# Arktis2022/Spiking-Diffusion

Measured on AMD Instinct MI355X. Metric: images/sec + LIF-kernel HBM GB/s, MNIST 100-step sample T=16, 1->8 GPU, higher is better.
Workload: dtype fp32-exact (4 fp6 digits x fp4 spikes on the block-scaled MFMA + certified decisions + exact 6-digit recomputation of flagged neurons)

## Files before the change

### spiking-diffusion_amd/csrc/den_mfma_fp6v2.hip

```cpp
#include "den_common.h"
#include "../../include/spkdiff.h"
#include <math.h>
#include <stdlib.h>
#include <type_traits>
#include <utility>

namespace {

typedef int v6i __attribute__((ext_vector_type(6)));
typedef int v8i __attribute__((ext_vector_type(8)));
typedef float v16f __attribute__((ext_vector_type(16)));

constexpr int T16 = 16;
constexpr int CK = 32;
constexpr int POSB = T16 * CK / 2;
constexpr int WT = 64 * 24;
constexpr int N_PAIR = 18;
constexpr int N_D4 = 5;
constexpr int N_MAIN = N_PAIR + N_D4;
constexpr int N_L5 = 2;
constexpr int NACC = 2;
constexpr int W_PIECES = (N_PAIR * WT + 1023) / 1024;
constexpr int W_LDS = W_PIECES * 1024;
constexpr int W_SLAB = ((N_MAIN + N_L5) * WT + 1023) / 1024 * 1024;

constexpr unsigned FLAG_CAP = 1u << 20;

struct V2Args {
  const uint8_t* in0; int nch;
  const uint8_t* wq; const double* scale; const double* bias; const float* wl1;
  const float* bn_a; const float* bn_b;
  uint8_t* out; uint8_t* out_cnt;
  unsigned* flags;
  unsigned flag_cap;
  long long ticket_idx;
  int handover;
  const int* qtab;
  const int* n_dyn;
  const uint8_t* need; const int* cls_cnt; const int* cls_list;
  int B, Cout, Cin;
  int gx, nsets;
};

#define SPK_FP6_PRE "s_nop 1\n\t"
#define SPK_MFMA2(CLS, acc, av, bv, sa, sb)                                                                          \
  asm volatile(SPK_FP6_PRE "v_mfma_scale_f32_32x32x64_f8f6f4 %0, %1, %2, %0, %3, %4 op_sel_hi:[0,0,0] cbsz:4 blgp:2"  \
               : "+" CLS(acc) : "v"(av), "v"(bv), "v"(sa), "v"(sb))
#define SPK_MFMA2_Z(CLS, acc, av, bv, sa, sb)                                                                        \
  asm volatile(SPK_FP6_PRE "v_mfma_scale_f32_32x32x64_f8f6f4 %0, %1, %2, 0, %3, %4 op_sel_hi:[0,0,0] cbsz:4 blgp:2"   \
               : "=&" CLS(acc) : "v"(av), "v"(bv), "v"(sa), "v"(sb))

constexpr int SPK_V2_KMIN = 2;
constexpr float SPK_V2_SPARE = 1.0f;
constexpr int SPK_V2_REC_STEP = 13;
constexpr int SPK_V2_LP_PAIRS = 1;
constexpr int SPK_V2_GX_KB = 2560;
constexpr int SPK_V2_HALF_FILL = 2;
constexpr int SPK_V2_LPS_MIN_B = 64;
constexpr int SPK_V2_LP_SPLIT_MAX = 512;
constexpr int SPK_V2_PF = 6;

constexpr float CERT_4EPS = 4.0f * 2.38418579e-07f;

__device__ __forceinline__ void store_tile_spikes(uint8_t* out, uint8_t* out_cnt, unsigned mybits, int lane, long long rec_base,
                                                  long long cnt_base, bool ok) {
  const unsigned bitsv = spk_transpose16_rows(mybits, lane);
  if (out_cnt && ok) out_cnt[cnt_base + (lane & 31)] = (uint8_t)__popc(mybits);
  if (ok) *reinterpret_cast<uint2*>(out + rec_base + (lane & 15) * 16 + 8 * ((lane >> 4) & 1)) = spk_e2m1_record(bitsv);
}

__device__ const uint8_t V2_HALF_REC[2][64] = {
    {0, 1, 2, 3, 4, 5, 6, 7, 8, 9, 10, 11, 12, 13, 14, 15, 16, 17, 18, 19, 20, 21, 22, 23,
     23, 23, 23, 23, 23, 23, 23, 23, 23, 23, 23, 23, 23, 23, 23, 23, 23, 23, 23, 23, 23, 23, 23, 23, 24},
    {24, 25, 26, 27, 28, 29, 30, 31, 32, 33, 34, 35, 36, 37, 38, 39, 40, 41, 42, 43, 44, 45, 46, 47,
     47, 47, 47, 47, 47, 47, 47, 47, 47, 47, 47, 47, 47, 47, 47, 47, 47, 47, 47, 47, 47, 47, 47, 47, 24}};

enum : int { V2_INT = 0, V2_TOP, V2_RIGHT, V2_LEFT, V2_BOTTOM, V2_NCLS };
struct V2Plan { int nblk; int tap[9]; int nt[9]; };
constexpr int V2_FT = 3;
constexpr V2Plan V2_PLAN[V2_NCLS] = {
    {9, {0, 1, 2, 3, 4, 5, 6, 7, 8}, {3, 3, 3, 3, 3, 3, 3, 3, 3}},
    {6, {3, 4, 5, 6, 7, 8}, {3, 3, 3, 3, 3, 3}},
    {6, {0, 1, 3, 4, 6, 7}, {3, 3, 3, 3, 3, 3}},
    {6, {1, 2, 4, 5, 7, 8}, {3, 3, 3, 3, 3, 3}},
    {9, {0, 6, 7, 8, 1, 2, 3, 4, 5}, {3, 1, 1, 1, 3, 3, 3, 3, 3}}};
constexpr V2Plan v2_uniform_plan(int nt) {
  V2Plan p = {9, {0, 1, 2, 3, 4, 5, 6, 7, 8}, {}};
  for (int b = 0; b < 9; ++b) p.nt[b] = nt;
  return p;
}
constexpr int v2_plan_start(const V2Plan& p, int blk) {
  int n = 0;
  for (int b = 0; b < blk; ++b) n += p.nt[b];
  return n;
}
constexpr int v2_plan_blk(const V2Plan& p, int s) {
  int b = 0;
  while (s >= p.nt[b]) s -= p.nt[b++];
  return b;
}
__device__ constexpr uint8_t V2_FULL_POS[8][V2_FT][2] = {
    {{0, 1}, {2, 3}, {4, 5}},       {{6, 13}, {20, 27}, {34, 41}},  {{7, 14}, {21, 28}, {35, 42}},  {{43, 44}, {45, 46}, {47, 40}},
    {{8, 9}, {10, 11}, {12, 15}},   {{16, 17}, {18, 19}, {22, 23}}, {{24, 25}, {26, 29}, {30, 31}}, {{32, 33}, {36, 37}, {38, 39}}};
__device__ constexpr uint8_t V2_WAVE_CLS[8] = {V2_TOP, V2_RIGHT, V2_LEFT, V2_BOTTOM, V2_INT, V2_INT, V2_INT, V2_INT};
constexpr bool v2_full_map_ok() {
  bool seen[48] = {};
  for (int w = 0; w < 8; ++w)
    for (int i = 0; i < V2_FT; ++i)
      for (int h = 0; h < 2; ++h) {
        const int p = V2_FULL_POS[w][i][h];
        if (p >= 48 || seen[p]) return false;
        seen[p] = true;
      }
  for (int w = 0; w < 8; ++w) {
    const V2Plan& pl = V2_PLAN[V2_WAVE_CLS[w]];
    for (int i = 0; i < V2_FT; ++i)
      for (int tap = 0; tap < 9; ++tap) {
        int n = 0;
        for (int b = 0; b < pl.nblk; ++b) n += pl.tap[b] == tap && i >= V2_FT - pl.nt[b];
        if (n > 1) return false;
        for (int h = 0; h < 2 && n == 0; ++h) {
          const int y = V2_FULL_POS[w][i][h] / 7 + tap / 3 - 1, x = V2_FULL_POS[w][i][h] % 7 + tap % 3 - 1;
          if (y >= 0 && y < 7 && x >= 0 && x < 7) return false;
        }
      }
  }
  return true;
}
static_assert(v2_full_map_ok(), "full 7x7 items: position table and block lists");

template <int H, int W, int NWV, bool SPLIT, int NTP, bool HALF = false, int CLS = V2_INT>
__device__ __forceinline__ void fp6v2_body(const V2Args& a, const int g, const int il, const int lanes, const int n_images,
                                           const int* __restrict__ slots) {
  constexpr bool PRUNE = NTP > 0;
  static_assert(!HALF || (PRUNE && !SPLIT && H == 7 && W == 7 && NWV == 4 && NTP == 3), "half-image items: 7x7, four waves x three tiles");
  constexpr bool REC = !PRUNE;
  constexpr int HW = H * W, PW = W + 1;
  constexpr int Hb = SPLIT ? H / 2 : H;
  constexpr int Hin = SPLIT ? Hb + 1 : H;
  constexpr int HWb = Hb * W;
  static_assert(SPLIT ? ((H % 2) == 0 && (HWb % (2 * NWV)) == 0)
                      : ((HW & 1) == 1 && ((HW / 2) % NWV) == 0), "whole 32-row tiles on every wave (+ one odd position)");
  static_assert(!PRUNE || (!SPLIT && (NWV == 4 || NWV == 8) && NTP <= (HWb / 2) / NWV), "position lists: 7x7 items");
  constexpr int NT = PRUNE ? NTP : (HWb / 2) / NWV;
  constexpr int N_AGPR = NWV == 4 ? (NACC * NT < 16 ? NACC * NT : 16) : 0;
  constexpr int NPP = (Hin + 2) * PW + 1;
  constexpr int A_BYTES = NPP * POSB;
  constexpr int PPR = (W + 3) / 4;
  constexpr int NA = Hin * PPR;
  constexpr int NPA = (NA + NWV - 1) / NWV;
  constexpr int NPW = (W_PIECES + NWV - 1) / NWV;
  constexpr bool BSKIP = NWV == 8 && !PRUNE && !SPLIT;
  static_assert(!BSKIP || (H == 7 && W == 7 && NT == V2_FT), "border skip: the position table is for 7x7 items of three tiles per wave");
  static_assert(BSKIP || CLS == V2_INT, "wave classes: full 7x7 items only");
  static_assert(NWV >= 8 || NACC * NT <= 16 || (NT - 1) * NACC <= N_AGPR + 2, "only the last tile may straddle the register files");
  constexpr bool AH = NWV == 8 && !PRUNE;
  constexpr int NBUF = 2;
  extern __shared__ __attribute__((aligned(16))) uint8_t lds[];
  uint8_t* const sA = lds;
  uint8_t* const sW = lds + NBUF * A_BYTES;
  int* const s_cin = reinterpret_cast<int*>(lds + NBUF * A_BYTES + NBUF * W_LDS);
  int* const s_row = s_cin + NPP * 16;
  int* const s_nmax = s_row + (HWb + 1) * 16;
  const unsigned sA_addr = spk_lds_addr(sA), sW_addr = sA_addr + NBUF * A_BYTES;
  const int tid = threadIdx.x, lane = tid & 63, wave = tid >> 6;
  const int nch = a.nch;
  const int G = a.Cout >> 5;
  for (int i = tid; i < NBUF * A_BYTES / 16; i += NWV * 64) reinterpret_cast<uint4*>(sA)[i] = make_uint4(0, 0, 0, 0);
  if (REC)
    for (int i = tid; i < NPP * 16; i += NWV * 64) s_cin[i] = 0;
  __syncthreads();

  const int row = lane & 31, half = lane >> 5;
  const int hsel = (row >> 2) & 1, tt = (row & 3) + 4 * (row >> 3);
  int a_off[NT];
  int p_out[NT];
#pragma unroll
  for (int i = 0; i < NT; ++i) {
    const int p = BSKIP ? (int)V2_FULL_POS[wave & 7][i % V2_FT][hsel] : 2 * (wave + NWV * i) + hsel;
    a_off[i] = ((p / W) * PW + (p % W)) * POSB + tt * 16;
    p_out[i] = BSKIP ? (int)V2_FULL_POS[wave & 7][i % V2_FT][half] : 2 * (wave + NWV * i) + half;
  }

  const int wave_s = __builtin_amdgcn_readfirstlane(wave);
  unsigned pa_pk[NPA];
#pragma unroll
  for (int j = 0; j < NPA; ++j) {
    int id = wave_s * NPA + j;
    id = id < NA ? id : NA - 1;
    const int y = id / PPR, px = id - y * PPR;
    const int np = (W - 4 * px) < 4 ? (W - 4 * px) : 4;
    const unsigned src = (unsigned)((y * W + 4 * px) * POSB), dst = (unsigned)(((y + 1) * PW + 1 + 4 * px) * POSB);
    pa_pk[j] = src | (dst << 14) | ((unsigned)(np - 1) << 29);
  }
  const unsigned lane16 = (unsigned)lane * 16u;
  const unsigned wave_k = (unsigned)wave_s * 1024u;
  auto issue_piece = [&](int q, const uint8_t* aslab, const uint8_t* wslab, unsigned dA, unsigned dW) {
    if (q < NPA) {
      const unsigned pk = pa_pk[q];
      const unsigned np = ((pk >> 29) & 3u) + 1u;
      const unsigned long long mask = np == 4 ? ~0ull : ((1ull << (16 * np)) - 1ull);
      spk_dma16s_masked(aslab + (pk & 0x3fffu), lane16, dA + ((pk >> 14) & 0x7fffu), mask);
    } else {
      unsigned ko = wave_k + 1024u * NWV * (unsigned)(q - NPA);
      if (NWV * (q - NPA) + NWV - 1 >= W_PIECES) ko = ko < (unsigned)W_PIECES * 1024u ? ko : ko - 1024u * NWV;
      spk_dma16s(wslab + ko, lane16, dW + ko);
    }
  };
  const uint8_t* const wbase = a.wq + (long long)g * nch * W_SLAB;
  auto aslab_of = [&](int itm, int c) -> const uint8_t* {
    const int b = HALF ? itm >> 1 : (PRUNE ? slots[itm] : (SPLIT ? itm >> 1 : itm)), band = SPLIT ? itm & 1 : 0;
    return a.in0 + ((long long)b * nch + c) * HW * POSB + band * (Hb - 1) * W * POSB;
  };
  const int nitems = (SPLIT || HALF) ? 2 * n_images : n_images;

  const int co = g * 32 + (lane & 31);
  const float scale_f = (float)a.scale[co], bias_f = (float)a.bias[co];
  const float bna = a.bn_a[co], bnb = a.bn_b[co];
  const float Bc = fmaf(bias_f, bna, bnb);
  const float cE = 2.0f * 2.38418579e-07f * (fabsf(bnb) + fabsf(Bc)) + 1e-30f;
  const float cT = 528.0f * scale_f * fabsf(bna) * 1.000001f;
  const float Ac4 = 1024.0f * scale_f * bna;

  const int sc_a = 0x7f7f7f7f;
  const int sc_p = half ? (int)0x82828282u : (int)0x87878787u;

  int it = 0;
  if (il < nitems) {
    const uint8_t* as0 = aslab_of(il, 0);
#pragma unroll
    for (int q = 0; q < NPA + NPW; ++q) issue_piece(q, as0, wbase, sA_addr, sW_addr);
    if constexpr (AH) {
      spk_dma_wait_all();
      __syncthreads();
    }
  }
  for (int itm = il; itm < nitems; itm += lanes) {
    const int b = HALF ? itm >> 1 : (PRUNE ? slots[itm] : (SPLIT ? itm >> 1 : itm)), band = SPLIT ? itm & 1 : 0;
    const int band_off = band * PW * POSB;
    int n_list = 2 * NT * NWV;
    if constexpr (PRUNE) {
      const uint8_t* rec = HALF ? &V2_HALF_REC[itm & 1][0] : a.need + (long long)b * 64;
      n_list = __builtin_amdgcn_readfirstlane((int)rec[48]);
#pragma unroll
      for (int i = 0; i < NT; ++i) {
        const int k2 = 2 * (wave + NWV * i);
        const int p = rec[k2 + hsel];
        a_off[i] = ((p / W) * PW + (p % W)) * POSB + tt * 16;
        p_out[i] = rec[k2 + half];
      }
    }
    v16f acc[NT][NACC];
    int cnt[NT];
#pragma unroll
    for (int i = 0; i < NT; ++i) cnt[i] = 0;
    constexpr int NREC = Hin * W * 16, NR = (NREC + NWV * 64 - 1) / (NWV * 64);
    int creg[NR];
    int rec_off[NR];
    bool rec_ok[NR];
#pragma unroll
    for (int k = 0; k < NR; ++k) {
      creg[k] = 0;
      const int r = tid + k * NWV * 64;
      const int cl = r >> 4, t = r & 15;
      rec_ok[k] = r < NREC;
      rec_off[k] = rec_ok[k] ? (((cl / W) + 1) * PW + 1 + (cl % W)) * POSB + t * 16 : 0;
    }
    constexpr int PFX = NWV == 4 ? SPK_V2_PF : 4;
    v6i bp[2][2];
    v4i af[PFX];
    for (int c = 0; c < nch; ++c, ++it) {
      const int buf = it & 1, buf1 = buf ^ 1;
      if constexpr (!AH) {
        spk_dma_wait_all();
        __syncthreads();
      }
      int nb = itm, nc = c + 1;
      if (nc == nch) { nc = 0; nb = itm + lanes; }
      const bool have_next = nb < nitems;
      const uint8_t* n_aslab = aslab_of(have_next ? nb : itm, have_next ? nc : c);
      const uint8_t* n_wslab = wbase + (long long)(have_next ? nc : c) * W_SLAB;
      const unsigned n_dA = sA_addr + buf1 * A_BYTES;
      const unsigned n_dW = sW_addr + buf1 * W_LDS;

      v4i rvq[NR];
      auto compute = [&](auto first_tag) {
        constexpr bool FIRST = decltype(first_tag)::value;
        const uint8_t* A = sA + buf * A_BYTES + band_off;
        const uint8_t* Wb = sW + buf * W_LDS;
        auto toff = [](int tap) constexpr -> int { return ((tap / 3) * PW + (tap % 3)) * POSB; };
        constexpr V2Plan P = BSKIP ? V2_PLAN[CLS] : v2_uniform_plan(NT);
        constexpr int NBLK = P.nblk, NSTEP = v2_plan_start(P, NBLK);
        constexpr int PF = PFX;
        constexpr int NPIECES = NPA + NPW;
        static_assert(P.nt[0] == NT, "the first block writes (not accumulates) every accumulator");
        static_assert(2 * NBLK >= NPIECES, "two copy slots per block: every DMA piece of the wave gets one");
        static_assert((!AH || NSTEP >= 2 * PF) && (!REC || NSTEP > SPK_V2_REC_STEP), "look-ahead slots; the record-count steps exist");
        static_assert(!AH || (v2_plan_start(P, (NPIECES + 1) / 2) <= NSTEP - PF && v2_plan_start(P, NBLK - 2) <= NSTEP - PF),
                      "chunk barrier behind the copies and the last weight-tile read");
        auto lda_at = [&](const uint8_t* base, auto s_tag) -> v4i {
          constexpr int s = decltype(s_tag)::value;
          constexpr int blk = v2_plan_blk(P, s), i = NT - P.nt[blk] + (s - v2_plan_start(P, blk));
          return *reinterpret_cast<const v4i*>(base + a_off[i] + toff(P.tap[blk]));
        };
        auto lda = [&](auto s_tag) -> v4i { return lda_at(A, s_tag); };
        auto ldb = [&](int tile) -> v6i {
          const uint8_t* p = Wb + tile * WT;
          const v4i x = *reinterpret_cast<const v4i*>(p + lane * 16);
          typedef const volatile __attribute__((address_space(3))) v2i* lds_v2i_ptr;
          const v2i y = *(lds_v2i_ptr)SPK_LDS(p + 1024 + lane * 8);
          const v6i r = {x[0], x[1], x[2], x[3], y[0], y[1]};
          return r;
        };
        if constexpr (!AH || FIRST) {
          bp[0][0] = ldb(2 * P.tap[0]); bp[0][1] = ldb(2 * P.tap[0] + 1);
          static_for<PF>([&](auto s_tag) { af[decltype(s_tag)::value] = lda(s_tag); });
        }
        const uint8_t* An = sA + buf1 * A_BYTES + band_off;
        const uint8_t* Wn = sW + buf1 * W_LDS;
        const bool ahead = AH && c + 1 < nch;
        static_for<NSTEP>([&](auto s_tag) {
          constexpr int s = decltype(s_tag)::value;
          constexpr int blk = v2_plan_blk(P, s), nt = P.nt[blk], j = s - v2_plan_start(P, blk);
          constexpr int i = NT - nt + j;
          if constexpr (AH && s == NSTEP - PF) {
            asm volatile("s_waitcnt vmcnt(0)\n\ts_barrier" ::: "memory");
          }
          const v4i av = af[s % PF];
          if constexpr (s + PF < NSTEP) af[s % PF] = lda(std::integral_constant<int, s + PF>{});
          else if constexpr (AH) {
            constexpr int k = s % PF;
            if (ahead) af[k] = lda_at(An, std::integral_constant<int, k>{});
          }
#define V2_DMA_SLOT()                                                                              \
  do {                                                                                             \
    if constexpr (j == 0 && 2 * blk < NPIECES) issue_piece(2 * blk, n_aslab, n_wslab, n_dA, n_dW);     \
    if constexpr (j == (nt > 1 ? nt / 2 : 0) && 2 * blk + 1 < NPIECES)                             \
      issue_piece(2 * blk + 1, n_aslab, n_wslab, n_dA, n_dW);                                      \
  } while (0)
#define V2_NEXT_TILES()                                                                            \
  do {                                                                                             \
    if constexpr (j == 0 && blk + 1 < NBLK) {                                                      \
      bp[(blk + 1) & 1][0] = ldb(2 * P.tap[(blk + 1) % 9]);                                        \
      bp[(blk + 1) & 1][1] = ldb(2 * P.tap[(blk + 1) % 9] + 1);                                    \
    }                                                                                              \
  } while (0)
          if constexpr (!REC) {
            asm volatile("v_bcnt_u32_b32 %0, %1, %0\n\tv_bcnt_u32_b32 %0, %2, %0\n\tv_bcnt_u32_b32 %0, %3, %0\n\t"
                         "v_bcnt_u32_b32 %0, %4, %0" : "+v"(cnt[i]) : "v"(av[0]), "v"(av[1]), "v"(av[2]), "v"(av[3]));
          }
#define V2_PAIR_MFMA(J)                                                                                      \
do {                                                                                                        \
  if constexpr (FIRST && blk == 0) {                                                                        \
    if constexpr (NACC * i + (J) < N_AGPR) SPK_MFMA2_Z("a", acc[i][J], av, bp[0][J], sc_a, sc_p);              \
    else SPK_MFMA2_Z("v", acc[i][J], av, bp[0][J], sc_a, sc_p);                                             \
  } else {                                                                                                  \
    if constexpr (NACC * i + (J) < N_AGPR) SPK_MFMA2("a", acc[i][J], av, bp[blk & 1][J], sc_a, sc_p);          \
    else SPK_MFMA2("v", acc[i][J], av, bp[blk & 1][J], sc_a, sc_p);                                         \
  }                                                                                                         \
} while (0)
          V2_PAIR_MFMA(0);
          __builtin_amdgcn_sched_barrier(0);
          V2_DMA_SLOT();
          V2_NEXT_TILES();
          if constexpr (REC) {
            if constexpr (s == 1) {
#pragma unroll
              for (int k = 0; k < NR; ++k) rvq[k] = *reinterpret_cast<const v4i*>(sA + buf * A_BYTES + rec_off[k]);
            }
            if constexpr (s == SPK_V2_REC_STEP) {
#pragma unroll
              for (int k = 0; k < NR; ++k)
                creg[k] += __builtin_popcount((unsigned)rvq[k][0]) + __builtin_popcount((unsigned)rvq[k][1]) +
                           __builtin_popcount((unsigned)rvq[k][2]) + __builtin_popcount((unsigned)rvq[k][3]);
            }
          }
          V2_PAIR_MFMA(1);
          __builtin_amdgcn_sched_barrier(0);
          if constexpr (AH && s == NSTEP - 1) {
            if (ahead) {
              auto ldb_n = [&](int tile) -> v6i {
                const uint8_t* p = Wn + tile * WT;
                const v4i x = *reinterpret_cast<const v4i*>(p + lane * 16);
                typedef const volatile __attribute__((address_space(3))) v2i* lds_v2i_ptr;
                const v2i y = *(lds_v2i_ptr)SPK_LDS(p + 1024 + lane * 8);
                const v6i r = {x[0], x[1], x[2], x[3], y[0], y[1]};
                return r;
              };
              bp[0][0] = ldb_n(2 * P.tap[0]); bp[0][1] = ldb_n(2 * P.tap[0] + 1);
            }
          }
        });
      };
      if (c == 0) compute(std::true_type{}); else compute(std::false_type{});
    }

    if constexpr (REC) {
#pragma unroll
      for (int k = 0; k < NR; ++k)
        if (rec_ok[k]) s_cin[(rec_off[k] / POSB) * 16 + ((rec_off[k] % POSB) >> 4)] = creg[k];
      if (tid <= HWb) s_nmax[tid] = 0;
      __syncthreads();
      for (int e = tid; e < HWb * 16; e += NWV * 64) {
        const int pp = e >> 4, t = e & 15;
        const int* c0 = s_cin + (((pp / W) + band) * PW + (pp % W)) * 16 + t;
        int sum = 0;
#pragma unroll
        for (int dy = 0; dy < 3; ++dy)
#pragma unroll
          for (int dx = 0; dx < 3; ++dx) sum += c0[(dy * PW + dx) * 16];
        s_row[e] = sum;
        atomicMax(&s_nmax[pp], sum);
      }
      __syncthreads();
    }
    asm volatile("s_nop 15\n\ts_nop 15" ::: "memory");

#pragma unroll
    for (int k = 0; k < NT; ++k) {
      const int i = k == 0 ? NT - 1 : k - 1;
#pragma unroll
      for (int j = 0; j < NACC; ++j)
        if (NACC * i + j < N_AGPR) asm volatile("" : "+a"(acc[i][j]));
      float v = 0.f;
      unsigned mybits = 0;
      bool flg = false;
      int cntv[16];
      if constexpr (!REC) {
#pragma unroll
        for (int r = 0; r < 16; ++r) {
          const int rowA = (r & 3) + 8 * (r >> 2);
          const int c0 = __builtin_amdgcn_readlane(cnt[i], rowA), c1 = __builtin_amdgcn_readlane(cnt[i], rowA + 4);
          cntv[r] = half ? c1 : c0;
        }
      }
      int nmax_rec = 0;
      if constexpr (REC) nmax_rec = s_nmax[BSKIP ? p_out[i] : 2 * (wave + NWV * i) + half];
      typedef float v2f __attribute__((ext_vector_type(2)));
      float zmax = 0.f, dmin = 3.0e38f;
      int nmax = nmax_rec;
#pragma unroll
      for (int r2 = 0; r2 < 16; r2 += 2) {
        const v2f p0 = {acc[i][0][r2], acc[i][0][r2 + 1]}, p1 = {acc[i][1][r2], acc[i][1][r2 + 1]};
        const v2f q4 = __builtin_elementwise_fma(p0, (v2f){1024.0f, 1024.0f}, p1);
        const v2f z2 = __builtin_elementwise_fma(q4, (v2f){Ac4, Ac4}, (v2f){Bc, Bc});
        if constexpr (!REC) nmax = max(nmax, max(cntv[r2], cntv[r2 + 1]));
#pragma unroll
        for (int e = 0; e < 2; ++e) {
          const float z = z2[e];
          zmax = fmaxf(zmax, fabsf(z));
          const float h = fmaf(z - v, 0.5f, v);
          const float hm = h - 1.0f;
          dmin = fminf(dmin, fabsf(hm));
          const bool s = h >= 1.0f;
          v = s ? 0.0f : h;
          mybits = __builtin_amdgcn_alignbit(mybits, __float_as_uint(hm), 31);
        }
      }
      mybits = ~(__builtin_bitreverse32(mybits) >> 16) & 0xffffu;
      flg = dmin <= SPK_V2_SPARE * fmaf(zmax, 2.5f * CERT_4EPS, fmaf((float)nmax, cT, cE));
      if (__builtin_amdgcn_ballot_w64(flg) != 0ull) {
        float v2 = 0.f, dh = 0.f;
        bool f2 = false;
        if constexpr (REC) {
          const v4i* rp = reinterpret_cast<const v4i*>(s_row + (BSKIP ? p_out[i] : 2 * (wave + NWV * i) + half) * 16);
#pragma unroll
          for (int q = 0; q < 4; ++q) {
            const v4i c4 = rp[q];
            cntv[4 * q] = c4[0]; cntv[4 * q + 1] = c4[1]; cntv[4 * q + 2] = c4[2]; cntv[4 * q + 3] = c4[3];
          }
        }
#pragma unroll
        for (int r2 = 0; r2 < 16; r2 += 2) {
          const v2f p0 = {acc[i][0][r2], acc[i][0][r2 + 1]}, p1 = {acc[i][1][r2], acc[i][1][r2 + 1]};
          const v2f q4 = __builtin_elementwise_fma(p0, (v2f){1024.0f, 1024.0f}, p1);
          const v2f z2 = __builtin_elementwise_fma(q4, (v2f){Ac4, Ac4}, (v2f){Bc, Bc});
#pragma unroll
          for (int e = 0; e < 2; ++e) {
            const float z = z2[e];
            const float ct = fmaf((float)cntv[r2 + e], cT, cE);
            dh = fmaf(fabsf(z) + fabsf(v2), 0.625f * CERT_4EPS, fmaf(dh, 0.5f, 0.5f * ct));
            const float h = fmaf(z - v2, 0.5f, v2);
            f2 = f2 || (fabsf(h - 1.0f) <= SPK_V2_SPARE * dh);
            v2 = h >= 1.0f ? 0.0f : h;
          }
        }
        flg = flg && f2;
      }
      const int ti = wave + NWV * i;
      const int p = (PRUNE || BSKIP) ? p_out[i] : 2 * ti + half + band * HWb;
      const bool listed = !PRUNE || 2 * ti + half < n_list;
      if (flg && listed) {
        const long long n = ((long long)b * a.Cout + co) * HW + p;
        const unsigned idx = atomicAdd(a.flags, 1u);
        if (idx < a.flag_cap) a.flags[2 + idx] = (unsigned)n;
        else atomicOr(a.flags + 2 + FLAG_CAP + (n >> 5), 1u << (n & 31));
      }
      const long long rec = (((long long)b * G + g) * HW + p) * POSB;
      store_tile_spikes(a.out, a.out_cnt, mybits, lane, rec, (((long long)b * G + g) * HW + p) * 32, listed);
      __builtin_amdgcn_sched_barrier(0);
    }
  }
  spk_dma_wait_all();
}

__device__ __forceinline__ void fp6v2_wg_map(const V2Args& a, int& g, int& il, int& lanes) {
  const int k = blockIdx.x, G = a.Cout >> 5;
  if (a.gx > 0) {
    const int S = gridDim.x >> 3, x = k & 7, slot = k >> 3;
    const int npart = 8 / a.nsets, set = x % a.nsets, xi = x / a.nsets, lanes_x = S / a.gx;
    g = set * a.gx + slot % a.gx;
    il = xi * lanes_x + slot / a.gx;
    lanes = npart * lanes_x;
  } else {
    g = k % G;
    il = k / G;
    lanes = gridDim.x / G;
  }
}

__device__ __forceinline__ void fp6v2_handover(const V2Args& a) {
  if (!a.handover) return;
  __syncthreads();
  if (threadIdx.x == 0) {
    if (atomicAdd(a.flags + a.ticket_idx, 1u) == gridDim.x - 1) {
      a.flags[1] = atomicAdd(a.flags, 0u);
      a.flags[0] = 0u;
      a.flags[a.ticket_idx] = 0u;
    }
  }
}


template <int H, int W, int NWV, bool SPLIT = false>
__global__ __launch_bounds__(NWV * 64, 1) void conv3x3_fp6v2_kernel(V2Args a) {
  const int Bn = a.n_dyn ? (*a.n_dyn < a.B ? *a.n_dyn : a.B) : a.B;
  int g, il, lanes;
  fp6v2_wg_map(a, g, il, lanes);
  if constexpr (NWV == 8 && !SPLIT) {
    switch (__builtin_amdgcn_readfirstlane((int)V2_WAVE_CLS[(threadIdx.x >> 6) & 7])) {
      case V2_TOP: fp6v2_body<H, W, NWV, false, 0, false, V2_TOP>(a, g, il, lanes, Bn, nullptr); break;
      case V2_RIGHT: fp6v2_body<H, W, NWV, false, 0, false, V2_RIGHT>(a, g, il, lanes, Bn, nullptr); break;
      case V2_LEFT: fp6v2_body<H, W, NWV, false, 0, false, V2_LEFT>(a, g, il, lanes, Bn, nullptr); break;
      case V2_BOTTOM: fp6v2_body<H, W, NWV, false, 0, false, V2_BOTTOM>(a, g, il, lanes, Bn, nullptr); break;
      default: fp6v2_body<H, W, NWV, false, 0, false, V2_INT>(a, g, il, lanes, Bn, nullptr); break;
    }
  } else fp6v2_body<H, W, NWV, SPLIT, 0>(a, g, il, lanes, Bn, nullptr);
  fp6v2_handover(a);
}

template <int H, int W>
__global__ __launch_bounds__(256, 1) void conv3x3_fp6v2_half_kernel(V2Args a) {
  const int Bn = a.n_dyn ? (*a.n_dyn < a.B ? *a.n_dyn : a.B) : a.B;
  int g, il, lanes;
  fp6v2_wg_map(a, g, il, lanes);
  fp6v2_body<H, W, 4, false, 3, true>(a, g, il, lanes, Bn, nullptr);
  fp6v2_handover(a);
}

template <int H, int W, int NWV>
__global__ __launch_bounds__(NWV * 64, 1) void conv3x3_fp6v2_listed_kernel(V2Args a) {
  constexpr int NC = (H * W / 2) / 4;
  int g, il, lanes;
  fp6v2_wg_map(a, g, il, lanes);
  int cnt[NC], work[NC], u[NC];
  int total = 0, nonempty = 0;
#pragma unroll
  for (int k = 0; k < NC; ++k) {
    cnt[k] = a.cls_cnt[k];
    work[k] = cnt[k] * (k + 1 < SPK_V2_KMIN ? SPK_V2_KMIN : k + 1);
    total += work[k];
    nonempty += cnt[k] > 0;
  }
  if (total == 0) { fp6v2_handover(a); return; }
  int rem = lanes - nonempty, used = 0;
#pragma unroll
  for (int k = 0; k < NC; ++k) {
    u[k] = cnt[k] > 0 ? 1 + (int)((long long)rem * work[k] / total) : 0;
    used += u[k];
  }
  for (int left = lanes - used; left > 0; --left) {
    int best = 0;
    long long bw = -1, bu = 1;
#pragma unroll
    for (int k = 0; k < NC; ++k)
      if (cnt[k] > 0 && (long long)work[k] * bu > bw * u[k]) { bw = work[k]; bu = u[k]; best = k; }
#pragma unroll
    for (int k = 0; k < NC; ++k) u[k] += (k == best);
  }
  int start = 0, cls = -1, il_c = 0, lanes_c = 1;
#pragma unroll
  for (int k = 0; k < NC; ++k) {
    if (il >= start && il < start + u[k]) { cls = k; il_c = il - start; lanes_c = u[k]; }
    start += u[k];
  }
  const int* slots = a.cls_list + (long long)(cls < 0 ? 0 : cls) * a.B;
  static_assert(NWV == 8, "listed positions: two waves per SIMD");
  switch (cls) {
    case 0: case 1: fp6v2_body<H, W, 8, false, 1>(a, g, il_c, lanes_c, cnt[cls], slots); break;
    case 2: case 3: fp6v2_body<H, W, 8, false, 2>(a, g, il_c, lanes_c, cnt[cls], slots); break;
    case 4: case 5: fp6v2_body<H, W, 8, false, 3>(a, g, il_c, lanes_c, cnt[cls], slots); break;
    default: break;
  }
  fp6v2_handover(a);
}

__device__ __forceinline__ float exact_preact(double s, double sc, double bi) { return (float)fma(s, sc, bi); }

template <int H, int W, bool WIDE>
__device__ __forceinline__ void fp6v2_lastpos_body(const V2Args& a, const int bid, float (*red)[16][64]) {
  constexpr int HW = H * W, NP = SPK_V2_LP_PAIRS;
  const int lane = threadIdx.x & 63, wave = threadIdx.x >> 6;
  const int nch = a.nch, G = a.Cout >> 5;
  const int Bn = a.n_dyn ? (*a.n_dyn < a.B ? *a.n_dyn : a.B) : a.B;
  if (!a.handover && bid == 0 && threadIdx.x == 0) { a.flags[1] = a.flags[0]; a.flags[0] = 0u; }
  const int n_units = ((Bn + 2 * NP - 1) / (2 * NP)) * G;
  const bool split = n_units <= SPK_V2_LP_SPLIT_MAX;
  const int unit = split ? bid : bid * 4 + wave;
  const int g = unit % G, b0 = (unit / G) * 2 * NP;
  if (b0 >= Bn) return;
  const int row = lane & 31, half = lane >> 5;
  const int hsel = (row >> 2) & 1, tt = (row & 3) + 4 * (row >> 3);
  const int sc_a = 0x7f7f7f7f;
  const int sc_p = half ? (int)0x82828282u : (int)0x87878787u;
  const int sc_hi = (int)0x87878787u, sc_lo = (int)0x82828282u;
  v16f acc[NP][3];
#pragma unroll
  for (int q = 0; q < NP; ++q)
#pragma unroll
    for (int j = 0; j < 3; ++j)
#pragma unroll
      for (int r = 0; r < 16; ++r) acc[q][j][r] = 0.f;
  const int py = H - 1, px = W - 1;
  for (int c = split ? wave : 0; c < nch; c += split ? 4 : 1) {
    const uint8_t* wslab = a.wq + ((long long)g * nch + c) * W_SLAB;
    auto ldb = [&](int tile) -> v8i {
      const uint8_t* wt = wslab + tile * WT;
      const v4i bx = *reinterpret_cast<const v4i*>(wt + lane * 16);
      const v2i by = *reinterpret_cast<const v2i*>(wt + 1024 + lane * 8);
      return v8i{bx[0], bx[1], bx[2], bx[3], by[0], by[1], 0, 0};
// ... 566 lines not shown
```

Before: 3267.

## Assign DMA copy roles to three waves for full 7x7 items

For full 7x7 items processed by eight waves, the activation and weight DMA pieces are no longer spread across all waves. Only three waves copy activations and three copy weights, the wave index comes from the compile-time border class, and the first weight slab is issued before the LDS zeroing. In the main loop the copies go into one slot per step instead of two slots per block. The aim is fewer copy instructions on most waves and an earlier first weight load, at the cost of uneven per-wave copy load and a more complex schedule guarded by constexpr ownership checks.

```diff
diff --git a/spiking-diffusion_amd/csrc/den_mfma_fp6v2.hip b/spiking-diffusion_amd/csrc/den_mfma_fp6v2.hip
--- a/spiking-diffusion_amd/csrc/den_mfma_fp6v2.hip
+++ b/spiking-diffusion_amd/csrc/den_mfma_fp6v2.hip
@@ -129,6 +129,45 @@
 }
 static_assert(v2_full_map_ok(), "full 7x7 items: position table and block lists");
 
+constexpr int V2_FULL_NCA = 3, V2_FULL_NCWW = 3;
+constexpr int v2_ceil_div(int a, int b) { return (a + b - 1) / b; }
+constexpr int v2_copy_na(int na, int ncw, int w) {
+  const int npa = v2_ceil_div(na, ncw), left = na - w * npa;
+  return w >= ncw || left <= 0 ? 0 : (left < npa ? left : npa);
+}
+constexpr int v2_copy_nw(int nw, int ncw, int w) {
+  return w >= ncw || w >= nw ? 0 : (nw - w + ncw - 1) / ncw;
+}
+constexpr int v2_rec_off(int r, int nrec, int w) {
+  const int cl = r >> 4, t = r & 15;
+  return r < nrec ? (((cl / w) + 1) * (w + 1) + 1 + (cl % w)) * POSB + t * 16 : 0;
+}
+constexpr bool v2_roles_ok(int nwv, int nca, int ncww, int na, int nw, int nrec, int w) {
+  int pa[64] = {}, pw[64] = {};
+  if (na > 64 || nw > 64 || nca > nwv || ncww > nwv) return false;
+  for (int wv = 0; wv < nwv; ++wv) {
+    for (int j = 0; j < v2_copy_na(na, nca, wv); ++j) ++pa[wv * v2_ceil_div(na, nca) + j];
+    for (int q = 0; q < v2_copy_nw(nw, ncww, wv); ++q) ++pw[wv + ncww * q];
+  }
+  for (int i = 0; i < na; ++i) if (pa[i] != 1) return false;
+  for (int i = 0; i < nw; ++i) if (pw[i] != 1) return false;
+  const int nct = 64 * nwv, nr = v2_ceil_div(nrec, nct);
+  int seen[1024] = {};
+  if (nrec > 1024) return false;
+  for (int tid = 0; tid < nct; ++tid)
+    for (int k = 0; k < nr; ++k) {
+      const int r = tid + k * nct, off = v2_rec_off(r, nrec, w);
+      if (r < nrec) {
+        const int cell = off / POSB, y = cell / (w + 1), x = cell % (w + 1);
+        if (y < 1 || x < 1 || x > w || (y - 1) * w + (x - 1) != (r >> 4) || (off % POSB) != (r & 15) * 16) return false;
+        ++seen[r];
+      } else if (off != 0) return false;
+    }
+  for (int r = 0; r < nrec; ++r) if (seen[r] != 1) return false;
+  return true;
+}
+static_assert(v2_roles_ok(8, V2_FULL_NCA, V2_FULL_NCWW, 7 * 2, W_PIECES, 7 * 7 * 16, 7), "full 7x7 items: 41 pieces, 784 records, one owner each");
+
 template <int H, int W, int NWV, bool SPLIT, int NTP, bool HALF = false, int CLS = V2_INT>
 __device__ __forceinline__ void fp6v2_body(const V2Args& a, const int g, const int il, const int lanes, const int n_images,
                                            const int* __restrict__ slots) {
@@ -148,11 +187,17 @@
   constexpr int A_BYTES = NPP * POSB;
   constexpr int PPR = (W + 3) / 4;
   constexpr int NA = Hin * PPR;
-  constexpr int NPA = (NA + NWV - 1) / NWV;
-  constexpr int NPW = (W_PIECES + NWV - 1) / NWV;
   constexpr bool BSKIP = NWV == 8 && !PRUNE && !SPLIT;
   static_assert(!BSKIP || (H == 7 && W == 7 && NT == V2_FT), "border skip: the position table is for 7x7 items of three tiles per wave");
   static_assert(BSKIP || CLS == V2_INT, "wave classes: full 7x7 items only");
+  constexpr int NCA = BSKIP ? V2_FULL_NCA : NWV, NCWW = BSKIP ? V2_FULL_NCWW : NWV;
+  constexpr bool KNOWN = BSKIP && CLS != V2_INT;
+  constexpr int CWV = KNOWN ? CLS - 1 : 0;
+  static_assert(!KNOWN || V2_WAVE_CLS[CWV] == CLS, "border class k is wave k - 1");
+  static_assert(!BSKIP || v2_roles_ok(NWV, NCA, NCWW, NA, W_PIECES, Hin * W * 16, W), "copy roles, record counting");
+  constexpr int NPA_T = (NA + NCA - 1) / NCA;
+  constexpr int NPA = KNOWN ? v2_copy_na(NA, NCA, CWV) : ((!BSKIP || NCA == NWV) ? NPA_T : 0);
+  constexpr int NPW = KNOWN ? v2_copy_nw(W_PIECES, NCWW, CWV) : ((!BSKIP || NCWW == NWV) ? (W_PIECES + NCWW - 1) / NCWW : 0);
   static_assert(NWV >= 8 || NACC * NT <= 16 || (NT - 1) * NACC <= N_AGPR + 2, "only the last tile may straddle the register files");
   constexpr bool AH = NWV == 8 && !PRUNE;
   constexpr int NBUF = 2;
@@ -166,6 +211,22 @@
   const int tid = threadIdx.x, lane = tid & 63, wave = tid >> 6;
   const int nch = a.nch;
   const int G = a.Cout >> 5;
+  const int wave_s = KNOWN ? CWV : __builtin_amdgcn_readfirstlane(wave);
+  const unsigned lane16 = (unsigned)lane * 16u;
+  const unsigned wave_k = (unsigned)wave_s * 1024u;
+  const uint8_t* const wbase = a.wq + (long long)g * nch * W_SLAB;
+  const int nitems = (SPLIT || HALF) ? 2 * n_images : n_images;
+  auto issue_w = [&](int qw, const uint8_t* wslab, unsigned dW) {
+    unsigned ko = wave_k + 1024u * NCWW * (unsigned)qw;
+    if (NCWW * qw + NCWW - 1 >= W_PIECES) ko = ko < (unsigned)W_PIECES * 1024u ? ko : ko - 1024u * NCWW;
+    spk_dma16s(wslab + ko, lane16, dW + ko);
+  };
+  if constexpr (BSKIP && NPW > 0) {
+    if (il < nitems) {
+#pragma unroll
+      for (int q = 0; q < NPW; ++q) issue_w(q, wbase, sW_addr);
+    }
+  }
   for (int i = tid; i < NBUF * A_BYTES / 16; i += NWV * 64) reinterpret_cast<uint4*>(sA)[i] = make_uint4(0, 0, 0, 0);
   if (REC)
     for (int i = tid; i < NPP * 16; i += NWV * 64) s_cin[i] = 0;
@@ -182,37 +243,28 @@
     p_out[i] = BSKIP ? (int)V2_FULL_POS[wave & 7][i % V2_FT][half] : 2 * (wave + NWV * i) + half;
   }
 
-  const int wave_s = __builtin_amdgcn_readfirstlane(wave);
-  unsigned pa_pk[NPA];
+  unsigned pa_pk[NPA > 0 ? NPA : 1];
 #pragma unroll
   for (int j = 0; j < NPA; ++j) {
-    int id = wave_s * NPA + j;
+    int id = wave_s * NPA_T + j;
     id = id < NA ? id : NA - 1;
     const int y = id / PPR, px = id - y * PPR;
     const int np = (W - 4 * px) < 4 ? (W - 4 * px) : 4;
     const unsigned src = (unsigned)((y * W + 4 * px) * POSB), dst = (unsigned)(((y + 1) * PW + 1 + 4 * px) * POSB);
     pa_pk[j] = src | (dst << 14) | ((unsigned)(np - 1) << 29);
   }
-  const unsigned lane16 = (unsigned)lane * 16u;
-  const unsigned wave_k = (unsigned)wave_s * 1024u;
   auto issue_piece = [&](int q, const uint8_t* aslab, const uint8_t* wslab, unsigned dA, unsigned dW) {
     if (q < NPA) {
       const unsigned pk = pa_pk[q];
       const unsigned np = ((pk >> 29) & 3u) + 1u;
       const unsigned long long mask = np == 4 ? ~0ull : ((1ull << (16 * np)) - 1ull);
       spk_dma16s_masked(aslab + (pk & 0x3fffu), lane16, dA + ((pk >> 14) & 0x7fffu), mask);
-    } else {
-      unsigned ko = wave_k + 1024u * NWV * (unsigned)(q - NPA);
-      if (NWV * (q - NPA) + NWV - 1 >= W_PIECES) ko = ko < (unsigned)W_PIECES * 1024u ? ko : ko - 1024u * NWV;
-      spk_dma16s(wslab + ko, lane16, dW + ko);
-    }
+    } else issue_w(q - NPA, wslab, dW);
   };
-  const uint8_t* const wbase = a.wq + (long long)g * nch * W_SLAB;
   auto aslab_of = [&](int itm, int c) -> const uint8_t* {
     const int b = HALF ? itm >> 1 : (PRUNE ? slots[itm] : (SPLIT ? itm >> 1 : itm)), band = SPLIT ? itm & 1 : 0;
     return a.in0 + ((long long)b * nch + c) * HW * POSB + band * (Hb - 1) * W * POSB;
   };
-  const int nitems = (SPLIT || HALF) ? 2 * n_images : n_images;
 
   const int co = g * 32 + (lane & 31);
   const float scale_f = (float)a.scale[co], bias_f = (float)a.bias[co];
@@ -229,7 +281,7 @@
   if (il < nitems) {
     const uint8_t* as0 = aslab_of(il, 0);
 #pragma unroll
-    for (int q = 0; q < NPA + NPW; ++q) issue_piece(q, as0, wbase, sA_addr, sW_addr);
+    for (int q = 0; q < (BSKIP ? NPA : NPA + NPW); ++q) issue_piece(q, as0, wbase, sA_addr, sW_addr);
     if constexpr (AH) {
       spk_dma_wait_all();
       __syncthreads();
@@ -262,9 +314,8 @@
     for (int k = 0; k < NR; ++k) {
       creg[k] = 0;
       const int r = tid + k * NWV * 64;
-      const int cl = r >> 4, t = r & 15;
       rec_ok[k] = r < NREC;
-      rec_off[k] = rec_ok[k] ? (((cl / W) + 1) * PW + 1 + (cl % W)) * POSB + t * 16 : 0;
+      rec_off[k] = v2_rec_off(r, NREC, W);
     }
     constexpr int PFX = NWV == 4 ? SPK_V2_PF : 4;
     v6i bp[2][2];
@@ -294,9 +345,10 @@
         constexpr int PF = PFX;
         constexpr int NPIECES = NPA + NPW;
         static_assert(P.nt[0] == NT, "the first block writes (not accumulates) every accumulator");
-        static_assert(2 * NBLK >= NPIECES, "two copy slots per block: every DMA piece of the wave gets one");
+        constexpr bool SLOT1 = BSKIP && (NCA != NWV || NCWW != NWV);
+        static_assert(SLOT1 || 2 * NBLK >= NPIECES, "two copy slots per block: every DMA piece of the wave gets one");
         static_assert((!AH || NSTEP >= 2 * PF) && (!REC || NSTEP > SPK_V2_REC_STEP), "look-ahead slots; the record-count steps exist");
-        static_assert(!AH || (v2_plan_start(P, (NPIECES + 1) / 2) <= NSTEP - PF && v2_plan_start(P, NBLK - 2) <= NSTEP - PF),
+        static_assert(!AH || ((SLOT1 ? NPIECES : v2_plan_start(P, (NPIECES + 1) / 2)) <= NSTEP - PF && v2_plan_start(P, NBLK - 2) <= NSTEP - PF),
                       "chunk barrier behind the copies and the last weight-tile read");
         auto lda_at = [&](const uint8_t* base, auto s_tag) -> v4i {
           constexpr int s = decltype(s_tag)::value;
@@ -334,8 +386,9 @@
           }
 #define V2_DMA_SLOT()                                                                              \
   do {                                                                                             \
-    if constexpr (j == 0 && 2 * blk < NPIECES) issue_piece(2 * blk, n_aslab, n_wslab, n_dA, n_dW);     \
-    if constexpr (j == (nt > 1 ? nt / 2 : 0) && 2 * blk + 1 < NPIECES)                             \
+    if constexpr (SLOT1 && s < NPIECES) issue_piece(s, n_aslab, n_wslab, n_dA, n_dW);                 \
+    if constexpr (!SLOT1 && j == 0 && 2 * blk < NPIECES) issue_piece(2 * blk, n_aslab, n_wslab, n_dA, n_dW);     \
+    if constexpr (!SLOT1 && j == (nt > 1 ? nt / 2 : 0) && 2 * blk + 1 < NPIECES)                   \
       issue_piece(2 * blk + 1, n_aslab, n_wslab, n_dA, n_dW);                                      \
   } while (0)
 #define V2_NEXT_TILES()                                                                            \
```

After: 3305, median of 6. 1.2% higher.
